# ushariRanasinghe/G2VLM

Measured on AMD Instinct MI355X. Metric: views/sec (multi-view recon, G2VLM-2B-MoT), higher is better.
Workload: dtype bf16; 1 GPU; C3: 8-view 518x518 reconstruction, full depth (24 DINO + 28 MoT + 15 decoder blocks), 1 scene per GPU; Lq=10968, Lk=10976, parallelism=replicas x1

## Files before the change

g2vlm_amd/csrc/gemm_8p.hip:

```cpp
#include <cstdlib>
#include "gemm_tile256.h"
#include "gemm_internal.h"

namespace {

typedef __attribute__((address_space(3))) void* lds_ptr_t;
typedef const __attribute__((address_space(1))) void* gbl_ptr_t;

template <int EPI, int MA0, int MA1, int PIPE>
__global__ __launch_bounds__(512, 2) void gemm8p_kernel(T256Args a) {
  constexpr int MT = MA0 + MA1;
  constexpr int HB = 16 * MT;
  constexpr int BMv = 2 * HB;
  constexpr int NA0 = (MA0 + 1) / 2, NA1 = (MA1 + 1) / 2;
  extern __shared__ __attribute__((aligned(16))) char smem[];

  const int tid = threadIdx.x, lane = tid & 63;
  const int w = __builtin_amdgcn_readfirstlane(tid >> 6);
  const int wr = w >> 2, wc = w & 3;
  const int N = a.N, K = a.K;
  const int srow = lane >> 3, scp = lane & 7;
  const int kcol = (scp ^ srow) << 3;
  int a_row[2][3], b_col[2][2], a_dst[2][3], b_dst[2][2];
#pragma unroll
  for (int q = 0; q < 2; ++q)
#pragma unroll
    for (int i2 = 0; i2 < 3; ++i2) {
      const int MA = q ? MA1 : MA0;
      int Lr = min(i2 * 64 + w * 8, 32 * MA - 8);
      a_row[q][i2] = (Lr / (16 * MA)) * HB + (q ? 16 * MA0 : 0) + Lr % (16 * MA);
      a_dst[q][i2] = a_row[q][i2] * 128;
    }
#pragma unroll
  for (int q = 0; q < 2; ++q)
#pragma unroll
    for (int i2 = 0; i2 < 2; ++i2) {
      int gq = w + 8 * i2;
      b_col[q][i2] = (gq >> 2) * 64 + q * 32 + (gq & 3) * 8;
      b_dst[q][i2] = OP_BYTES + b_col[q][i2] * 128;
    }

  struct TileCtx {
    int gi, m0, n0;
    uint32_t a_src[2][3], b_src[2][2];
  };
  auto setup_tile = [&](int vt, TileCtx& c) {
    tile_origin<BMv>(a, vt, c.gi, c.m0, c.n0);
    const int gM = a.g[c.gi].M;
#pragma unroll
    for (int q = 0; q < 2; ++q)
#pragma unroll
      for (int i2 = 0; i2 < 3; ++i2)
        c.a_src[q][i2] = ((uint32_t)(min(c.m0 + a_row[q][i2] + srow, gM - 1) - c.m0) * (uint32_t)a.lda + kcol) * 2u;
#pragma unroll
    for (int q = 0; q < 2; ++q)
#pragma unroll
      for (int i2 = 0; i2 < 2; ++i2)
        c.b_src[q][i2] = ((uint32_t)(min(c.n0 + b_col[q][i2] + srow, N - 1) - c.n0) * (uint32_t)K + kcol) * 2u;
  };
  auto stage_of = [&](int j, const __bf16* Ab, const __bf16* Wb, const uint32_t (&as)[2][3], const uint32_t (&bs)[2][2]) {
    const int t = j >> 2, c = j & 3;
    char* base = smem + (t & 1) * KBUF_BYTES;
    const char* Ak = reinterpret_cast<const char*>(Ab + t * BK);
    const char* Wk = reinterpret_cast<const char*>(Wb + t * BK);
    if (c == 0) {
#pragma unroll
      for (int i2 = 0; i2 < NA0; ++i2)
        if (i2 * 8 + w < 4 * MA0)
          __builtin_amdgcn_global_load_lds((gbl_ptr_t)(Ak + as[0][i2]), (lds_ptr_t)(base + a_dst[0][i2]), 16, 0, 0);
    } else if (c == 3) {
#pragma unroll
      for (int i2 = 0; i2 < NA1; ++i2)
        if (i2 * 8 + w < 4 * MA1)
          __builtin_amdgcn_global_load_lds((gbl_ptr_t)(Ak + as[1][i2]), (lds_ptr_t)(base + a_dst[1][i2]), 16, 0, 0);
    } else {
      const int q = c == 2;
#pragma unroll
      for (int i2 = 0; i2 < 2; ++i2)
        __builtin_amdgcn_global_load_lds((gbl_ptr_t)(Wk + bs[q][i2]), (lds_ptr_t)(base + b_dst[q][i2]), 16, 0, 0);
    }
  };

  TileCtx cur;
  setup_tile(blockIdx.x, cur);
  bool prefetched = false;
  for (int vt = blockIdx.x; vt < a.total; vt += gridDim.x) {
  const T256Group g = a.g[cur.gi];
  const int m0 = cur.m0, n0 = cur.n0, M = g.M;
  const __bf16* Abase = g.A + (size_t)m0 * a.lda;
  const __bf16* Wbase = g.W + (size_t)n0 * K;

  const int nk = K / BK;
  const int n_half = 4 * nk;
  auto stage = [&](int j) {
    if (j >= n_half || (prefetched && j < 4)) return;
    stage_of(j, Abase, Wbase, cur.a_src, cur.b_src);
  };
  auto wait_vm = [&](int n) {
    switch (n) {
      case 5: __builtin_amdgcn_s_waitcnt(0x0F75); break;
      case 6: __builtin_amdgcn_s_waitcnt(0x0F76); break;
      case 7: __builtin_amdgcn_s_waitcnt(0x0F77); break;
      case 8: __builtin_amdgcn_s_waitcnt(0x0F78); break;
      case 9: __builtin_amdgcn_s_waitcnt(0x0F79); break;
      default: __builtin_amdgcn_s_waitcnt(0x0F7A); break;
    }
  };
  const int cnt_a0 = (4 * MA0 - w + 7) >> 3, cnt_a1 = (4 * MA1 - w + 7) >> 3;
  auto wait_ring = [&]() { wait_vm(cnt_a0 + 4); };

  f32x4 acc[MT][4];
#pragma unroll
  for (int i = 0; i < MT; ++i)
#pragma unroll
    for (int j = 0; j < 4; ++j) acc[i][j] = f32x4{0.f, 0.f, 0.f, 0.f};

  const int fr = lane & 15, fq = lane >> 4;
  const int sw = (fq ^ (fr & 7)) << 4;
  const int aoff = (wr * HB + fr) * 128 + sw;
  const int boff = OP_BYTES + (wc * 64 + fr) * 128 + sw;

  bf16x8 fa[PIPE == 1 ? 2 : 1][MA0][2], fb[2][2][2];

  auto read_a = [&](const char* base, int qa) {
#pragma unroll
    for (int i = 0; i < (qa ? MA1 : MA0); ++i)
#pragma unroll
      for (int kk = 0; kk < 2; ++kk) {
#ifdef EXP_GEMM_HALF_LDS
        if (i & 1) { fa[PIPE == 1 ? qa : 0][i][kk] = fa[PIPE == 1 ? qa : 0][i - 1][kk]; continue; }
#endif
        fa[PIPE == 1 ? qa : 0][i][kk] = *reinterpret_cast<const bf16x8*>(base + ((aoff + (qa * 16 * MA0 + i * 16) * 128) ^ (kk << 6)));
      }
  };
  auto read_b = [&](const char* base, int qb) {
#pragma unroll
    for (int jj = 0; jj < 2; ++jj)
#pragma unroll
      for (int kk = 0; kk < 2; ++kk) {
#ifdef EXP_GEMM_HALF_LDS
        if (jj & 1) { fb[qb][jj][kk] = fb[qb][0][kk]; continue; }
#endif
        fb[qb][jj][kk] = *reinterpret_cast<const bf16x8*>(base + ((boff + qb * 4096 + jj * 2048) ^ (kk << 6)));
      }
  };
  const bool live = wr * HB < M - m0 || (a.flags & G2V_GEMM_8P_NO_ROW_SKIP);
  auto mma = [&](int qa, int qb) {
    if (!live) return;
#ifdef EXP_GEMM_NO_MFMA
#pragma unroll
    for (int kk = 0; kk < 2; ++kk) {
#pragma unroll
      for (int i = 0; i < (qa ? MA1 : MA0); ++i) acc[qa * MA0 + i][qb * 2][0] += (float)fa[PIPE == 1 ? qa : 0][i][kk][0];
#pragma unroll
      for (int jj = 0; jj < 2; ++jj) acc[qa * MA0][qb * 2 + jj][1] += (float)fb[qb][jj][kk][0];
    }
    return;
#endif
    __builtin_amdgcn_s_setprio(1);
#pragma unroll
    for (int kk = 0; kk < 2; ++kk)
#pragma unroll
      for (int i = 0; i < (qa ? MA1 : MA0); ++i)
#pragma unroll
        for (int jj = 0; jj < 2; ++jj)
          acc[qa * MA0 + i][qb * 2 + jj] =
              __builtin_amdgcn_mfma_f32_16x16x32_bf16(fb[qb][jj][kk], fa[PIPE == 1 ? qa : 0][i][kk], acc[qa * MA0 + i][qb * 2 + jj], 0, 0, 0);
    __builtin_amdgcn_s_setprio(0);
  };
  constexpr bool STAG = PIPE == 2;
  auto sync_lds = [&]() {
    if constexpr (STAG) {
      __builtin_amdgcn_s_waitcnt(0xC07F);
      __builtin_amdgcn_sched_barrier(0);
      __builtin_amdgcn_s_barrier();
    } else {
      __builtin_amdgcn_s_barrier();
      __builtin_amdgcn_s_waitcnt(0xC07F);
    }
    __builtin_amdgcn_sched_barrier(0);
  };

  if constexpr (PIPE != 1) {
    auto ktile = [&](int t) {
      const char* base = smem + (t & 1) * KBUF_BYTES;
      const int p = 4 * t;
      read_b(base, 0);
      __builtin_amdgcn_sched_barrier(0);
      read_a(base, 0);
      stage(p + 7);
      sync_lds();
      mma(0, 0);
      __builtin_amdgcn_s_barrier();
      read_b(base, 1);
      stage(p + 8);
      sync_lds();
      mma(0, 1);
      __builtin_amdgcn_s_barrier();
      read_a(base, 1);
      stage(p + 9);
      sync_lds();
      mma(1, 1);
      __builtin_amdgcn_s_barrier();
      stage(p + 10);
      if (t + 2 < nk) wait_ring();
      else __builtin_amdgcn_s_waitcnt(0x0F70);
      __builtin_amdgcn_s_barrier();
      mma(1, 0);
      __builtin_amdgcn_s_barrier();
    };

  #pragma unroll
    for (int j = 0; j < 7; ++j) stage(j);
    if (nk >= 2) wait_ring();
    else __builtin_amdgcn_s_waitcnt(0x0F70);
    __builtin_amdgcn_s_barrier();
    if constexpr (STAG) {
      if (wr == 1) __builtin_amdgcn_s_barrier();
    }

    for (int t = 0; t < nk; ++t) ktile(t);
    if constexpr (STAG) {
      if (wr == 0) __builtin_amdgcn_s_barrier();
    }
  } else {
    auto begin_phase = [&](bool retire, int t) {
      __builtin_amdgcn_s_waitcnt(0xC07F);
      if (retire && t + 1 < nk) {
        if (t + 2 < nk) wait_ring();
        else __builtin_amdgcn_s_waitcnt(0x0F70);
      }
      __builtin_amdgcn_sched_barrier(0);
      __builtin_amdgcn_s_barrier();
      __builtin_amdgcn_sched_barrier(0);
    };
#pragma unroll
    for (int j = 0; j < 8; ++j) stage(j);
    if (nk >= 2) {
      wait_vm(cnt_a0 + 4 + cnt_a1);
    } else {
      __builtin_amdgcn_s_waitcnt(0x0F70);
    }
    __builtin_amdgcn_s_barrier();
    read_a(smem, 0);
    read_b(smem, 0);
    __builtin_amdgcn_s_waitcnt(0xC07F);
    __builtin_amdgcn_s_barrier();
    stage(8);
    for (int t = 0; t < nk; ++t) {
      const char* base = smem + (t & 1) * KBUF_BYTES;
      const char* nbase = smem + ((t + 1) & 1) * KBUF_BYTES;
      const int p = 4 * t;
      begin_phase(false, t);
      stage(p + 9);
      read_b(base, 1);
      __builtin_amdgcn_sched_barrier(0);
      mma(0, 0);
      __builtin_amdgcn_sched_barrier(0);
      begin_phase(false, t);
      stage(p + 10);
      read_a(base, 1);
      __builtin_amdgcn_sched_barrier(0);
      mma(0, 1);
      __builtin_amdgcn_sched_barrier(0);
      begin_phase(true, t);
      stage(p + 11);
      read_a(nbase, 0);
      __builtin_amdgcn_sched_barrier(0);
      mma(1, 1);
      __builtin_amdgcn_sched_barrier(0);
      begin_phase(false, t);
      stage(p + 12);
      __builtin_amdgcn_sched_barrier(0);
      mma(1, 0);
      __builtin_amdgcn_sched_barrier(0);
      read_b(nbase, 0);
    }
    __builtin_amdgcn_s_waitcnt(0xC07F);
    __builtin_amdgcn_s_barrier();
  }

  const int vn = vt + gridDim.x;
  const bool has_next = vn < a.total;
  if (has_next) {
    setup_tile(vn, cur);
    const T256Group& gn_ = a.g[cur.gi];
    const __bf16* An = gn_.A + (size_t)cur.m0 * a.lda;
    const __bf16* Wn = gn_.W + (size_t)cur.n0 * K;
#pragma unroll
    for (int j = 0; j < 4; ++j) stage_of(j, An, Wn, cur.a_src, cur.b_src);
  }

#ifdef EXP_GEMM_NO_EPI
  {
    float sink = 0.f;
#pragma unroll
    for (int i = 0; i < MT; ++i)
#pragma unroll
      for (int j = 0; j < 4; ++j) sink += acc[i][j][0] + acc[i][j][1] + acc[i][j][2] + acc[i][j][3];
    if (sink == 1.2345e30f) reinterpret_cast<float*>(g.C)[tid] = sink;
    __builtin_amdgcn_s_barrier();
    prefetched = has_next;
    continue;
  }
#endif
  tile_epilogue<EPI, MT, 512, 4>(a, g, smem, tid, wr, wc, m0, n0, [&](auto i, auto j, auto r) { return acc[i.value][j.value][r.value]; });
  prefetched = has_next;
  }
}

template <int EPI, int MA0, int MA1, int PIPE>
int launch_h(const T256Args& a, hipStream_t s) { return launch_persistent<gemm8p_kernel<EPI, MA0, MA1, PIPE>, 512>(a, s); }

template <int EPI>
int launch(const T256Args& a, int bm, hipStream_t s) {
  if (a.flags & G2V_GEMM_8P_TWO_BARRIER) {
    if (bm == 288) return launch_h<EPI, 5, 4, 0>(a, s);
    if (bm == 256) return launch_h<EPI, 4, 4, 0>(a, s);
    if (bm == 224) return launch_h<EPI, 4, 3, 0>(a, s);
    if (bm == 192) return launch_h<EPI, 4, 2, 0>(a, s);
    if (bm == 160) return launch_h<EPI, 3, 2, 0>(a, s);
    return launch_h<EPI, 2, 2, 0>(a, s);
  }
  if (a.flags & G2V_GEMM_8P_PIPELINED) {
    if (bm == 288) return launch_h<EPI, 5, 4, 0>(a, s);
    if (bm == 256) return launch_h<EPI, 4, 4, 1>(a, s);
    if (bm == 224) return launch_h<EPI, 4, 3, 1>(a, s);
    if (bm == 192) return launch_h<EPI, 4, 2, 1>(a, s);
    if (bm == 160) return launch_h<EPI, 3, 2, 1>(a, s);
    return launch_h<EPI, 2, 2, 1>(a, s);
  }
  if (bm == 288) return launch_h<EPI, 5, 4, 2>(a, s);
  if (bm == 256) return launch_h<EPI, 4, 4, 2>(a, s);
  if (bm == 224) return launch_h<EPI, 4, 3, 2>(a, s);
  if (bm == 192) return launch_h<EPI, 4, 2, 2>(a, s);
  if (bm == 160) return launch_h<EPI, 3, 2, 2>(a, s);
  return launch_h<EPI, 2, 2, 2>(a, s);
}

}

static bool aligned16(const void* p) { return (reinterpret_cast<uintptr_t>(p) & 15) == 0; }

bool g2v_gemm_8p_supported(const g2v_gemm_desc* d) {
  if ((d->K % BK) || (d->N % BN) || (d->lda & 7) || d->K < 2 * BK) return false;
  if ((long)BM_MAX * d->lda >= (1L << 31) || (long)BN * d->K >= (1L << 31)) return false;
  const bool f32out = d->epilogue == G2V_EPI_RES_F32;
  if (d->ldc % (f32out ? 4 : 8)) return false;
  for (int i = 0; i < d->ngroups; ++i) {
    const g2v_gemm_group& g = d->g[i];
    if (g.M <= 0) continue;
    if (!aligned16(g.A) || !aligned16(g.W) || !aligned16(g.C)) return false;
    if (g.bias && (reinterpret_cast<uintptr_t>(g.bias) & 7)) return false;
    if (g.gamma && !aligned16(g.gamma)) return false;
    if (g.res && (!aligned16(g.res) || d->ldres % (f32out ? 4 : 8))) return false;
  }
  return true;
}

bool g2v_gemm_8p_preferred(const g2v_gemm_desc* d) {
  long rows = 0;
  for (int i = 0; i < d->ngroups; ++i) rows += d->g[i].M;
  return rows >= 1024 || (rows >= 256 && d->N >= 4096);
}

int g2v_gemm_8p_height(const g2v_gemm_desc* d) {
  const int tiles_n = d->N / BN;
  const int big = d->ngroups == 2 && d->g[1].M > d->g[0].M ? 1 : 0;
  const long m_big = d->g[big].M;
  const long m_small = d->ngroups == 2 ? d->g[1 - big].M : 0;
  int bm = 256;
  {
    double best = 1e30;
    const int hs[6] = {288, 256, 224, 192, 160, 128};
    const double hc[6] = {1.005, 1.0, 1.08, 1.12, 1.165, 1.23};
    for (int k = 0; k < 6; ++k) {
      const int h = hs[k];
      const int small_rows = m_small > 0 ? (int)((m_small + h - 1) / h) : 0;
      const long tiles = ((m_big + h - 1) / h + small_rows) * tiles_n;
      const long rounds = (tiles + 255) / 256;
      const double c = (double)rounds * h * hc[k];
      if (c < best) { best = c; bm = h; }
    }
  }
  if (d->flags & G2V_GEMM_8P_H192) bm = 192;
  if (d->flags & G2V_GEMM_8P_H128) bm = 128;
  if (d->flags & G2V_GEMM_8P_H256) bm = 256;
  if (d->flags & G2V_GEMM_8P_H288) bm = 288;
  if (d->flags & G2V_GEMM_8P_H224) bm = 224;
  if (d->flags & G2V_GEMM_8P_H160) bm = 160;
  return bm;
}

bool g2v_gemm_8p_four_waves(const g2v_gemm_desc* d) {
  if (d->flags & (G2V_GEMM_8P_EIGHT_WAVES | G2V_GEMM_8P_TWO_BARRIER | G2V_GEMM_8P_PIPELINED)) return false;
  static int mask = -1;
  if (mask < 0) {
    const char* e = getenv("G2V_GEMM_4W_MASK");
    mask = e ? atoi(e) : 6;
  }
  const int cls = d->N >= 8192 ? 1 : (d->K >= 4096 ? 2 : (d->epilogue == G2V_EPI_RES_F32 ? 4 : (d->epilogue == G2V_EPI_GELU ? 16 : 8)));
  return (d->flags & G2V_GEMM_8P_FOUR_WAVES) || (mask & cls);
}

int g2v_gemm_8p_launch(const g2v_gemm_desc* d, hipStream_t s) {
  const int bm = g2v_gemm_8p_height(d);
  T256Args a;
  a.ngroups = 0; a.N = d->N; a.K = d->K; a.lda = d->lda; a.ldc = d->ldc; a.ldres = d->ldres;
  a.tiles_n = d->N / BN; a.flags = d->flags;
  a.sn = a.tiles_n < 8 ? a.tiles_n : 8;
  a.sm = 32 / a.sn > 1 ? 32 / a.sn : 1;
  a.total = 0;
  const int big = d->ngroups == 2 && d->g[1].M > d->g[0].M;
  for (int i = 0; i < d->ngroups; ++i) {
    const g2v_gemm_group& sg = d->g[i ^ big];
    if (sg.M <= 0) continue;
    T256Group& g = a.g[a.ngroups++];
    g.A = (const __bf16*)sg.A; g.W = (const __bf16*)sg.W; g.bias = (const __bf16*)sg.bias; g.C = sg.C; g.res = sg.res;
    g.gamma = (const float*)sg.gamma; g.M = sg.M; g.tile_start = a.total;
    a.total += ((sg.M + bm - 1) / bm) * a.tiles_n;
  }
  if (a.ngroups == 1) a.g[1] = a.g[0];
  if (a.total == 0) return G2V_OK;
  if (g2v_gemm_8p_four_waves(d)) return g2v_gemm_4w_launch(a, d->epilogue, bm, s);
  return g2v_gemm_with_epilogue(d->epilogue, [&](auto epi) { return launch<decltype(epi)::value>(a, bm, s); });
}
```

g2vlm_amd/csrc/gemm_tile256.h:

```cpp
#pragma once
#include <type_traits>
#include <utility>
#include "common.h"
#include "g2vlm_hip.h"

struct T256Group {
  const __bf16* A; const __bf16* W; const __bf16* bias; void* C; const void* res; const float* gamma;
  int M, tile_start;
};
struct T256Args {
  T256Group g[2];
  int ngroups, N, K, lda, ldc, ldres, tiles_n, flags, sm, sn, total;
};

inline int g2v_persistent_cus() {
  static int n_cu = 0;
  if (n_cu == 0) {
    int dev = 0;
    hipDeviceProp_t prop;
    if (hipGetDevice(&dev) != hipSuccess || hipGetDeviceProperties(&prop, dev) != hipSuccess) return 0;
    n_cu = prop.multiProcessorCount & ~7;
    if (n_cu <= 0) n_cu = 256;
  }
  return n_cu;
}

namespace {

constexpr int BN = 256, BK = 64;
constexpr int BM_MAX = 288;
constexpr int OP_BYTES = BM_MAX * 128;
constexpr int KBUF_BYTES = OP_BYTES + 256 * 128;
constexpr int OUT_PITCH = 256 * 2 + 16;
constexpr int LDS_BYTES = KBUF_BYTES + 160 * OUT_PITCH;

template <class F, int... I>
__device__ __forceinline__ void sfor_impl(F&& f, std::integer_sequence<int, I...>) { (f(std::integral_constant<int, I>{}), ...); }
template <int N, class F>
__device__ __forceinline__ void sfor(F&& f) { sfor_impl(f, std::make_integer_sequence<int, N>{}); }

template <int BM>
__device__ __forceinline__ void tile_origin(const T256Args& a, int vt, int& gi, int& m0, int& n0) {
  const int nwg = a.total;
  int bid = vt;
  {
    int xcd = bid & 7, qn = nwg >> 3, rn = nwg & 7;
    bid = (xcd < rn ? xcd * (qn + 1) : rn * (qn + 1) + (xcd - rn) * qn) + (bid >> 3);
  }
  gi = (a.ngroups > 1 && bid >= a.g[1].tile_start) ? 1 : 0;
  const int t_id = bid - a.g[gi].tile_start;
  const int tiles_m = (a.g[gi].M + BM - 1) / BM;
  const int row_sz = a.sm * a.tiles_n;
  int sup_m = t_id / row_sz, r = t_id - sup_m * row_sz;
  int h = min(a.sm, tiles_m - sup_m * a.sm);
  int full_w = a.sn * h;
  int sup_n = r / full_w, p = r - sup_n * full_w;
  m0 = (sup_m * a.sm + p % h) * BM;
  n0 = (sup_n * a.sn + p / h) * BN;
}

template <int EPI, int MT, int NT, int NJ, class Acc>
__device__ __forceinline__ void tile_epilogue(const T256Args& a, const T256Group& g, char* smem, int tid, int wr, int wc, int m0, int n0, Acc&& acc) {
  constexpr bool SWI = EPI == G2V_EPI_SWIGLU;
  constexpr int HB = 16 * MT;
  constexpr int PITCH = OUT_PITCH;
  constexpr int I0 = (MT + 1) / 2;
  constexpr int CPR = SWI ? 16 : 32;
  constexpr int RPI = NT / CPR;
  const int M = g.M;
  char* const img = smem + KBUF_BYTES;
  int etid = tid;
  asm volatile("" : "+v"(etid));
  const int efr = etid & 15, efq = (etid >> 4) & 3;
  const int ch = etid % CPR, r0 = etid / CPR;
  const int gn = (SWI ? (n0 >> 1) : n0) + ch * 8;
  const bool round_gamma = a.flags & G2V_GEMM_GAMMA_ROUND_BF16;
  using OutT = std::conditional_t<EPI == G2V_EPI_RES_F32, float, __bf16>;
  const char* const rd = img + r0 * PITCH + ch * 16;
  OutT* const cl = reinterpret_cast<OutT*>(g.C) + gn;
  const OutT* const rl = reinterpret_cast<const OutT*>(g.res) + gn;
  sfor<2>([&](auto h_) {
    constexpr int h = h_;
    const int irow0 = wr * 16 * I0 + efr;
    if constexpr (SWI) {
      sfor<I0>([&](auto ii_) {
        constexpr int ii = ii_, i = h * I0 + ii;
        if constexpr (i < MT) {
          sfor<NJ / 2>([&](auto jp_) {
            constexpr int jp = jp_;
            float o[4];
            sfor<4>([&](auto r_) {
              constexpr int r = r_;
              float gt = bfround(acc(std::integral_constant<int, i>{}, std::integral_constant<int, 2 * jp>{}, r_));
              float up = bfround(acc(std::integral_constant<int, i>{}, std::integral_constant<int, 2 * jp + 1>{}, r_));
              float sl = bfround(siluf_fast_(gt));
              o[r] = sl * up;
            });
            *reinterpret_cast<u32x2*>(img + (irow0 + ii * 16) * PITCH + (wc * NJ * 8 + jp * 16 + efq * 4) * 2) =
                u32x2{pack_bf16x2(o[0], o[1]), pack_bf16x2(o[2], o[3])};
          });
        }
      });
    } else {
      sfor<NJ>([&](auto j_) {
        constexpr int j = j_;
        const int cl = wc * NJ * 16 + j * 16 + efq * 4;
        float bv[4] = {0.f, 0.f, 0.f, 0.f};
        if (g.bias) {
          u32x2 bb = *reinterpret_cast<const u32x2*>(g.bias + n0 + cl);
          bv[0] = bits2f_lo(bb[0]); bv[1] = bits2f_hi(bb[0]); bv[2] = bits2f_lo(bb[1]); bv[3] = bits2f_hi(bb[1]);
        }
        sfor<I0>([&](auto ii_) {
          constexpr int ii = ii_, i = h * I0 + ii;
          if constexpr (i < MT) {
            float o[4];
            sfor<4>([&](auto r_) {
              constexpr int r = r_;
              float v = bfround(acc(std::integral_constant<int, i>{}, j_, r_) + bv[r]);
              if constexpr (EPI == G2V_EPI_GELU) v = gelu_fast(v);
              if constexpr (EPI == G2V_EPI_QUICKGELU) {
                float u = bfround(1.702f * v);
                float sg = bfround(sigmoidf_(u));
                v = v * sg;
              }
              o[r] = v;
            });
            *reinterpret_cast<u32x2*>(img + (irow0 + ii * 16) * PITCH + cl * 2) = u32x2{pack_bf16x2(o[0], o[1]), pack_bf16x2(o[2], o[3])};
          }
        });
      });
    }
    float gam[8];
    bool has_gam = false;
    if constexpr (EPI == G2V_EPI_RES_F32) {
      has_gam = g.gamma != nullptr;
      if (has_gam) {
        f32x4 g0 = *reinterpret_cast<const f32x4*>(g.gamma + gn), g1 = *reinterpret_cast<const f32x4*>(g.gamma + gn + 4);
#pragma unroll
        for (int e = 0; e < 4; ++e) { gam[e] = g0[e]; gam[4 + e] = g1[e]; }
      }
    }
    __syncthreads();
    constexpr int NIT = 2 * 16 * I0 / RPI;
    constexpr int SB = NIT % 5 == 0 ? 5 : (NIT % 4 == 0 ? 4 : (NIT % 3 == 0 ? 3 : 2));
    static_assert(NIT % SB == 0, "sweep batches");
#pragma unroll
    for (int it0 = 0; it0 < NIT; it0 += SB) {
      u32x4 pk[SB];
      int gmv[SB];
      bool ok[SB];
      [[maybe_unused]] f32x4 ra[SB], rb[SB];
      [[maybe_unused]] u32x4 rr[SB];
#pragma unroll
      for (int c = 0; c < SB; ++c) {
        const int irow = (it0 + c) * RPI + r0;
        const int iwr = irow / (16 * I0), rem = irow - iwr * (16 * I0);
        const int trow = h * 16 * I0 + rem;
        gmv[c] = m0 + iwr * HB + trow;
        ok[c] = trow < HB && gmv[c] < M;
        if constexpr (EPI == G2V_EPI_RES_F32) {
          ra[c] = rb[c] = f32x4{0.f, 0.f, 0.f, 0.f};
          if (ok[c] && g.res) {
            const float* rp = rl + (size_t)gmv[c] * a.ldres;
            ra[c] = *reinterpret_cast<const f32x4*>(rp); rb[c] = *reinterpret_cast<const f32x4*>(rp + 4);
          }
        } else if constexpr (EPI == G2V_EPI_RES_BF16) {
          rr[c] = u32x4{0u, 0u, 0u, 0u};
          if (ok[c]) rr[c] = *reinterpret_cast<const u32x4*>(rl + (size_t)gmv[c] * a.ldres);
        }
      }
#pragma unroll
      for (int c = 0; c < SB; ++c) pk[c] = *reinterpret_cast<const u32x4*>(rd + (it0 + c) * RPI * PITCH);
#pragma unroll
      for (int c = 0; c < SB; ++c) {
        if (!ok[c]) continue;
        const int gm = gmv[c];
        if constexpr (EPI == G2V_EPI_RES_F32) {
          float v[8];
#pragma unroll
          for (int e = 0; e < 4; ++e) { v[2 * e] = bits2f_lo(pk[c][e]); v[2 * e + 1] = bits2f_hi(pk[c][e]); }
          if (has_gam) {
#pragma unroll
            for (int e = 0; e < 8; ++e) {
              v[e] = __fmul_rn(v[e], gam[e]);
              if (round_gamma) v[e] = bfround(v[e]);
            }
          }
          float* cp = cl + (size_t)gm * a.ldc;
          *reinterpret_cast<f32x4*>(cp) = f32x4{__fadd_rn(ra[c][0], v[0]), __fadd_rn(ra[c][1], v[1]), __fadd_rn(ra[c][2], v[2]), __fadd_rn(ra[c][3], v[3])};
          *reinterpret_cast<f32x4*>(cp + 4) = f32x4{__fadd_rn(rb[c][0], v[4]), __fadd_rn(rb[c][1], v[5]), __fadd_rn(rb[c][2], v[6]), __fadd_rn(rb[c][3], v[7])};
        } else if constexpr (EPI == G2V_EPI_RES_BF16) {
          u32x4 ov;
#pragma unroll
          for (int e = 0; e < 4; ++e)
            ov[e] = pack_bf16x2(bits2f_lo(rr[c][e]) + bits2f_lo(pk[c][e]), bits2f_hi(rr[c][e]) + bits2f_hi(pk[c][e]));
          *reinterpret_cast<u32x4*>(cl + (size_t)gm * a.ldc) = ov;
        } else {
          *reinterpret_cast<u32x4*>(cl + (size_t)gm * a.ldc) = pk[c];
        }
      }
    }
    __syncthreads();
  });
}

template <auto KERNEL, int NT>
int launch_persistent(const T256Args& a, hipStream_t s) {
  static bool attr_set = false;
  if (!attr_set) {
    if (hipFuncSetAttribute(reinterpret_cast<const void*>(KERNEL), hipFuncAttributeMaxDynamicSharedMemorySize, LDS_BYTES) != hipSuccess)
      return G2V_ERR_LAUNCH;
    attr_set = true;
  }
  const int n_cu = g2v_persistent_cus();
  if (n_cu == 0) return G2V_ERR_LAUNCH;
  hipLaunchKernelGGL(KERNEL, dim3(a.total < n_cu ? a.total : n_cu), dim3(NT), LDS_BYTES, s, a);
  G2V_CHECK_LAUNCH();
  return G2V_OK;
}

}
```

g2vlm_amd/hip.py:

```python
import ctypes as C
import os
import threading

import torch

_HERE = os.path.dirname(os.path.abspath(__file__))
LIB_PATH = os.environ.get("G2V_LIB_PATH") or os.path.join(_HERE, "lib", "libg2vlm_hip.so")

EPI_BF16, EPI_GELU, EPI_QUICKGELU, EPI_SWIGLU, EPI_RES_F32, EPI_RES_BF16 = range(6)
GAMMA_ROUND_BF16 = 1
FORCE_SMALL_TILE = 2
SUPERTILE = 4
FORCE_BIG_TILE = 8
FORCE_8P = 16
P8_H192, P8_H128, P8_H256, P8_TWO_BARRIER, P8_H288, P8_H224, P8_H160 = 128, 256, 512, 1024, 4096, 8192, 16384
P8_PIPELINED = 32768
P8_FOUR_WAVES = 65536
P8_EIGHT_WAVES = 131072
P8_NO_ROW_SKIP = 262144
F32, BF16 = 0, 1
NO_CAUSAL = 2 ** 30
_DEBUG_GEMM_FLAGS = int(os.environ.get("G2V_GEMM_FLAGS", "0"))


class GemmGroup(C.Structure):
    _fields_ = [("A", C.c_void_p), ("W", C.c_void_p), ("bias", C.c_void_p), ("C", C.c_void_p),
                ("res", C.c_void_p), ("gamma", C.c_void_p), ("M", C.c_int32), ("_pad", C.c_int32)]


class GemmDesc(C.Structure):
    _fields_ = [("g", GemmGroup * 2), ("ngroups", C.c_int32), ("N", C.c_int32), ("K", C.c_int32),
                ("lda", C.c_int32), ("ldc", C.c_int32), ("ldres", C.c_int32), ("epilogue", C.c_int32),
                ("flags", C.c_int32), ("workspace", C.c_void_p), ("workspace_bytes", C.c_int64)]


_P, _I, _F, _L = C.c_void_p, C.c_int, C.c_float, C.c_int64
_SIGS = {
    "g2v_version": ([], C.c_int),
    "g2v_arch": ([], C.c_char_p),
    "g2v_gemm_bf16": ([C.POINTER(GemmDesc), _P], C.c_int),
    "g2v_gemm_route": ([C.POINTER(GemmDesc), C.POINTER(C.c_int32 * 4)], C.c_int),
    "g2v_gemm_f32": ([_P, _P, _P, _P, _P, _I, _I, _I, _I, _I, _I, _I, _P], C.c_int),
    "g2v_layernorm": ([_P, _I, _I, _P, _P, _F, _P, _I, _I, _I, _I, _P], C.c_int),
    "g2v_rmsnorm": ([_P, _I, _P, _P, _I, _F, _P, _I, _I, _I, _I, _P], C.c_int),
    "g2v_mrope_table": ([_P, _I, _P, _P, _P, _P], C.c_int),
    "g2v_qknorm_mrope_cache": ([_P, _I, _I, _I, _P, _P, _P, _P, _I, _F, _I, _P, _P, _P, _P, _P, _P, _P], C.c_int),
    "g2v_flash_attn": ([_P, _I, _P, _I, _P, _I, _P, _I, _P, _I, _I, _I, _I, _F, _P, _P, _I, _P, _I, _I, _P, _P], C.c_int),
    "g2v_flash_attn_workspace": ([_I], C.c_int64),
    "g2v_debug_attn_form": ([_I], C.c_int),
    "g2v_rope2d": ([_P, _I, _I, _I, _I, _I, _P, _P, _P, _I, _P], C.c_int),
    "g2v_rope_vision": ([_P, _I, _I, _I, _I, _P, _P, _P], C.c_int),
    "g2v_im2col14": ([_P, _I, _I, _I, _P, _I, _P], C.c_int),
    "g2v_dino_preprocess": ([_P, _I, _I, _I, _I, C.POINTER(C.c_float), C.POINTER(C.c_float), _P, _P, _P], C.c_int),
    "g2v_dino_assemble": ([_P, _P, _P, _P, _P, _I, _I, _I, _P], C.c_int),
    "g2v_im2col_patch": ([_P, _I, _I, _I, _I, _P, _I, _P], C.c_int),
    "g2v_qwen_patchify_u8": ([_P, _I, _I, _I, C.POINTER(C.c_float), C.POINTER(C.c_float), _P, _I, _P], C.c_int),
    "g2v_vit_assemble": ([_P, _P, _P, _P, _I, _I, _I, _I, _P], C.c_int),
    "g2v_gather_rows_f32": ([_P, _I, _P, _P, _I, _I, _I, _P], C.c_int),
    "g2v_scatter_rows_f32": ([_P, _I, _P, _P, _I, _I, _I, _P], C.c_int),
    "g2v_cast_f32_bf16": ([_P, _P, _L, _P], C.c_int),
    "g2v_cast_bf16_f32": ([_P, _P, _L, _P], C.c_int),
    "g2v_pts_epilogue": ([_P, _I, _I, _I, _I, _P, _P, _P, _P], C.c_int),
    "g2v_pixel_shuffle14": ([_P, _I, _I, _I, _I, _P, _P], C.c_int),
    "g2v_lanczos_resize_u8": ([_P, _I, _I, _I, _P, _I, _I, _P, _P, _P, _I, _P, _P, _I, _P], C.c_int),
    "g2v_pts_epilogue_ps": ([_P, _I, _I, _I, _I, _I, _P, _P, _P, _P], C.c_int),
    "g2v_pixel_shuffle": ([_P, _I, _I, _I, _I, _I, _P, _P], C.c_int),
    "g2v_camera_tail": ([_P, _I, _I, _P, _P, _P, _P, _P, _P, _P, _P, _P, _P], C.c_int),
    "g2v_argmax_bf16": ([_P, _I, _P, _P, _P], C.c_int),
    "g2v_gemv_bf16": ([_P, _P, _P, _P, _P, _I, _I, _P], C.c_int),
    "g2v_decode_attn_workspace": ([_I, _I], C.c_int64),
    "g2v_gemv_rmsnorm_bf16": ([_P, _P, _F, _P, _P, _P, _I, _I, _P], C.c_int),
    "g2v_gemv_swiglu_bf16": ([_P, _P, _P, _I, _I, _P], C.c_int),
    "g2v_gemv_rmsnorm_swiglu_bf16": ([_P, _P, _F, _P, _P, _I, _I, _P], C.c_int),
    "g2v_decode_attn": ([_P, _P, _P, _P, _I, _I, _I, _F, _P, _P], C.c_int),
    "g2v_swiglu_bf16": ([_P, _P, _I, _P], C.c_int),
    "g2v_decode_attn_dyn": ([_P, _P, _P, _P, _P, _I, _I, _I, _F, _P, _P], C.c_int),
    "g2v_decode_advance": ([_P, _P, _P, _P], C.c_int),
    "g2v_decode_attn_batch": ([_P, _P, _P, _P, _P, _I, _L, _I, _I, _I, _F, _P, _P], C.c_int),
    "g2v_decode_advance_batch": ([_P, _P, _P, _I, _P], C.c_int),
    "g2v_decode_attn_fused": ([_P, _P, _P, _F, _I, _P, _P, _P, _P, _P, _P, _I, _L, _I, _I, _I, _F, _P, _P], C.c_int),
    "g2v_argmax_rows_bf16": ([_P, _I, _I, _L, _P, _P, _P], C.c_int),
    "g2v_gemv_pg": ([_P, _P, _F, _P, _P, _P, _P, _I, _I, _I, _P], C.c_int),
    "g2v_gemv_pg_batch": ([_P, _P, _F, _P, _P, _P, _P, _I, _I, _I, _I, _P], C.c_int),
    "g2v_decode_attn_pg_workspace": ([_I, _I, _I], C.c_int64),
    "g2v_decode_attn_pg": ([_P, _P, _P, _F, _I, _P, _P, _P, _P, _P, _P, _I, _L, _I, _I, _I, _F, _P, _P], C.c_int),
    "g2v_sample_rows_bf16": ([_P, _I, _I, _L, _P, _P, _P, _P], C.c_int),
    "g2v_decode_attn_shared_workspace": ([_I, _I, _I, _I, _I], C.c_int64),
    "g2v_decode_attn_shared": ([_P, _P, _P, _F, _I, _P, _P, _P, _P, _I, _P, _P, _P, _I, _L, _I, _I, _I, _F, _P, _P, _P], C.c_int),
    "g2v_gemv_pg_fp8": ([_P, _P, _F, _P, _P, _P, _P, _P, _I, _I, _I, _P], C.c_int),
    "g2v_gemv_pg_batch_fp8": ([_P, _P, _F, _P, _P, _P, _P, _P, _I, _I, _I, _I, _P], C.c_int),
    "g2v_gemv_pg_route": ([_I, _I, _I, _I, _I, _I, C.POINTER(C.c_int32 * 4)], C.c_int),
    "g2v_kv_quant_e4m3": ([_P, _L, _I, _P, _P, _P], C.c_int),
    "g2v_kv_dequant_e4m3": ([_P, _P, _L, _I, _P, _P], C.c_int),
    "g2v_decode_attn_pg_kv8": ([_P, _P, _P, _F, _I, _P, _P, _P, _P, _P, _P, _P, _P, _I, _L, _I, _I, _I, _F, _P, _P], C.c_int),
    "g2v_logprob_rows_workspace": ([_I, _I], C.c_int64),
    "g2v_logprob_rows_bf16": ([_P, _I, _I, _L, _P, _P, _P, _P, _P, _L, _P], C.c_int),
    "g2v_topk_rows_workspace": ([_I, _I, _I], C.c_int64),
    "g2v_topk_rows_bf16": ([_P, _I, _I, _L, _I, _P, _P, _P, _L, _P], C.c_int),
}
EXPORTS = tuple(_SIGS)

_lib = None


def lib():
    global _lib
    if _lib is None:
        if not os.path.exists(LIB_PATH):
            raise RuntimeError(f"{LIB_PATH} is missing: run `python -m g2vlm_amd.build` (hipcc, gfx950). "
                               "g2vlm_amd has no CPU fallback.")
        _lib = C.CDLL(LIB_PATH)
        for name, (args, res) in _SIGS.items():
            fn = getattr(_lib, name)
            fn.argtypes, fn.restype = args, res
        if torch.cuda.is_available():
            want = _lib.g2v_arch().decode()
            have = getattr(torch.cuda.get_device_properties(torch.cuda.current_device()), "gcnArchName", "")
            if have and not have.split(":")[0] == want:
                _lib = None
                raise RuntimeError(f"libg2vlm_hip.so is built for {want}; this device is {have}")
        if os.environ.get("G2V_ATTN_FORM"):
            _lib.g2v_debug_attn_form(int(os.environ["G2V_ATTN_FORM"]))
    return _lib


class HipError(RuntimeError):
    pass


def _ck(rc, what):
    if rc != 0:
        raise HipError(f"{what} failed with code {rc}")


_raw_stream = getattr(torch._C, "_cuda_getCurrentRawStream", None)


def _stream():
    if _raw_stream is not None:
        return C.c_void_p(_raw_stream(torch.cuda.current_device()))
    return C.c_void_p(torch.cuda.current_stream().cuda_stream)


def _p(t):
    if t is None:
        return None
    assert t.is_cuda, "libg2vlm_hip takes device pointers only"
    return C.c_void_p(t.data_ptr())


def _rowmajor(t):
    assert t.dim() == 2 and t.stride(1) == 1, "row-major 2-D view expected"
    return t.stride(0)


def h2d(t, device, dtype=None, resident=False):
    if t.is_cuda:
        return t.to(dtype) if dtype is not None else t
    if dtype is not None:
        t = t.to(dtype)
    if torch.device(device).type != "cuda":
        return t.to(device)
    out = t.contiguous().pin_memory().to(device, non_blocking=True)
    if resident:
        torch.cuda.current_stream(out.device).synchronize()
    return out


def scratch_owner(device_index):
    return (device_index, int(torch._C._cuda_getCurrentRawStream(device_index)), threading.get_ident())


# ... 648 lines not shown
```

include/g2vlm_hip.h:

```cpp
#ifndef G2VLM_HIP_H
#define G2VLM_HIP_H
#include <stdint.h>
#ifdef __cplusplus
extern "C" {
#endif

int g2v_version(void);
const char* g2v_arch(void);

enum {
  G2V_EPI_BF16 = 0,
  G2V_EPI_GELU = 1,
  G2V_EPI_QUICKGELU = 2,
  G2V_EPI_SWIGLU = 3,
  G2V_EPI_RES_F32 = 4,
  G2V_EPI_RES_BF16 = 5
};
#define G2V_GEMM_GAMMA_ROUND_BF16 1
#define G2V_GEMM_SUPERTILE 4
#define G2V_GEMM_FORCE_BIG_TILE 8
#define G2V_GEMM_FORCE_8P 16
#define G2V_GEMM_8P_H192 128
#define G2V_GEMM_8P_H128 256
#define G2V_GEMM_8P_H256 512
#define G2V_GEMM_8P_TWO_BARRIER 1024
#define G2V_GEMM_8P_H288 4096
#define G2V_GEMM_8P_H224 8192
#define G2V_GEMM_8P_H160 16384
#define G2V_GEMM_8P_PIPELINED 32768
#define G2V_GEMM_8P_FOUR_WAVES 65536
#define G2V_GEMM_8P_NO_ROW_SKIP 262144
#define G2V_GEMM_8P_EIGHT_WAVES 131072
#define G2V_GEMM_FORCE_SMALL_TILE 2

typedef struct {
  const void* A;
  const void* W;
  const void* bias;
  void* C;
  const void* res;
  const void* gamma;
  int32_t M;
  int32_t _pad;
} g2v_gemm_group;

typedef struct {
  g2v_gemm_group g[2];
  int32_t ngroups, N, K, lda, ldc, ldres, epilogue, flags;
  void* workspace;
  int64_t workspace_bytes;
} g2v_gemm_desc;

int g2v_gemm_bf16(const g2v_gemm_desc* desc, void* stream);
int g2v_gemm_route(const g2v_gemm_desc* desc, int32_t out[4]);

int g2v_gemm_f32(const void* A, const void* W, const void* bias, void* C, const void* res,
                 int M, int N, int K, int lda, int ldc, int ldres, int relu, void* stream);

#define G2V_F32 0
#define G2V_BF16 1
int g2v_layernorm(const void* x, int x_dtype, int ldx, const void* w, const void* b, float eps,
                  void* out, int out_dtype, int ldo, int M, int C, void* stream);
int g2v_rmsnorm(const void* x, int ldx, const void* w_lo, const void* w_hi, int split, float eps,
                void* out, int out_dtype, int ldo, int M, int C, void* stream);

int g2v_mrope_table(const void* pos, int L, const void* inv_freq , void* cos, void* sin, void* stream);
int g2v_qknorm_mrope_cache(const void* qkv, int L, int Hq, int Hkv,
                           const void* qw_lo, const void* qw_hi, const void* kw_lo, const void* kw_hi,
                           int split, float eps, int und_rounding, const void* cos, const void* sin,
                           void* q_out, void* k_cache, void* v_cache, const void* kv_rows, void* stream);

typedef struct {
  int32_t q0, q_rows;
  int32_t k0, k_len;
  int32_t causal_shift;
  int32_t q_win0;
  int32_t _pad[2];
} g2v_attn_tile;

typedef struct {
  int32_t desc;
  int32_t head;
  int32_t kt0, kt1;
  int32_t slot;
  int32_t _pad[3];
} g2v_attn_seg;
int64_t g2v_flash_attn_workspace(int n_slots);
int g2v_debug_attn_form(int form);
int g2v_flash_attn(const void* q, int ldq, const void* k, int ldk, const void* v, int ldv,
                   void* o, int ldo, const g2v_attn_tile* tiles, int n_tiles,
                   int Hq, int Hkv, int D, float scale,
                   const g2v_attn_seg* segs, const int32_t* seg_ptr, int n_blocks, const int32_t* comb, int n_comb,
                   int tile_rows, void* workspace, void* stream);

int g2v_rope2d(void* x, int ld, int M, int col0, int n_heads, int D, const void* cos, const void* sin,
               const void* pos, int P, void* stream);

int g2v_rope_vision(void* x, int ld, int M, int n_heads, int D, const void* cos, const void* sin, void* stream);

int g2v_dino_preprocess(const void* in, int in_is_u8, int N, int H, int W, const float* mean3, const float* std3, void* norm,
                        void* orig, void* stream);

int g2v_lanczos_resize_u8(const void* src, int N, int Hin, int Win, void* dst, int Hout, int Wout, void* tmp,
                          const void* bounds_h, const void* kk_h, int ksize_h,
                          const void* bounds_v, const void* kk_v, int ksize_v, void* stream);
int g2v_im2col14(const void* img, int N, int H, int W, void* out, int Kpad, void* stream);
int g2v_dino_assemble(const void* patch, const void* cls, const void* regs, const void* pos,
                      void* x, int N, int P, int C, void* stream);

int g2v_im2col_patch(const void* img, int N, int H, int W, int patch, void* out, int Kpad, void* stream);
int g2v_vit_assemble(const void* patch, const void* cls, const void* regs, void* x, int N, int P, int R, int C,
                     void* stream);

int g2v_qwen_patchify_u8(const void* img_u8, int F, int H, int W, const float* mean3, const float* std3, void* out,
                         int Kpad, void* stream);

int g2v_gather_rows_f32(const void* src, int ld_src, const void* idx, void* dst, int ld_dst,
                        int rows, int C, void* stream);
int g2v_scatter_rows_f32(const void* src, int ld_src, const void* idx, void* dst, int ld_dst,
                         int rows, int C, void* stream);
int g2v_cast_f32_bf16(const void* src, void* dst, int64_t n, void* stream);
int g2v_cast_bf16_f32(const void* src, void* dst, int64_t n, void* stream);

int g2v_pts_epilogue_ps(const void* feat, int N, int H, int W, int patch, int mode, const void* pose,
                        void* out, void* out2, void* stream);
int g2v_pts_epilogue(const void* feat, int N, int H, int W, int mode, const void* pose,
                     void* out, void* out2, void* stream);
int g2v_pixel_shuffle(const void* feat, int N, int H, int W, int C, int patch, void* out, void* stream);
int g2v_pixel_shuffle14(const void* feat, int N, int H, int W, int C, void* out, void* stream);

int g2v_camera_tail(const void* feat, int N, int P, const void* w0, const void* b0, const void* w1,
                    const void* b1, const void* wt, const void* bt, const void* wr, const void* br,
                    void* pose, void* stream);

int g2v_argmax_bf16(const void* x, int n, void* out, void* scratch, void* stream);


int g2v_gemv_bf16(const void* x, const void* W, const void* bias, void* out, void* res, int N, int K, void* stream);
int g2v_gemv_rmsnorm_bf16(const void* x_f32, const void* norm_w, float eps, const void* W, const void* bias, void* out,
                          int N, int K, void* stream);
int g2v_gemv_swiglu_bf16(const void* gu, const void* W, void* res, int N, int K, void* stream);
int g2v_gemv_rmsnorm_swiglu_bf16(const void* x_f32, const void* norm_w, float eps, const void* W_gu, void* act_out,
                                 int N2, int K, void* stream);
int g2v_swiglu_bf16(const void* gu, void* out, int n, void* stream);
int64_t g2v_decode_attn_workspace(int Lk, int Hq);
int g2v_decode_attn(const void* q, const void* k_cache, const void* v_cache, void* out, int Lk, int Hq,
                    int Hkv, float scale, void* workspace, void* stream);
int g2v_decode_attn_dyn(const void* q, const void* k_cache, const void* v_cache, void* out, const void* Lk_dev,
                        int max_len, int Hq, int Hkv, float scale, void* workspace, void* stream);
int g2v_decode_advance(void* pos3, void* row, void* len, void* stream);

int g2v_decode_attn_batch(const void* q, const void* k_cache, const void* v_cache, void* out, const void* Lk_dev,
                          int batch, int64_t scene_rows, int max_len, int Hq, int Hkv, float scale, void* workspace,
                          void* stream);
int g2v_decode_attn_fused(const void* qkv, const void* q_norm_w, const void* k_norm_w, float eps, int und_rounding,
                          const void* cos, const void* sin, void* k_cache, void* v_cache, void* out, const void* Lk_dev,
                          int batch, int64_t scene_rows, int max_len, int Hq, int Hkv, float scale, void* workspace,
                          void* stream);
int g2v_decode_advance_batch(void* pos3, void* row, void* len, int batch, void* stream);
int g2v_argmax_rows_bf16(const void* x, int rows, int n, int64_t ld, void* out, void* scratch, void* stream);
int g2v_sample_rows_bf16(const void* x, int rows, int n, int64_t ld, void* out, void* scratch, void* rng, void* stream);


int g2v_gemv_pg(const void* x, const void* norm_w, float eps, const void* W, const void* bias, void* out, void* res, int N,
                int K, int act, void* stream);
int g2v_gemv_pg_batch(const void* x, const void* norm_w, float eps, const void* W, const void* bias,
                      void* out, void* res, int B, int N, int K, int act, void* stream);

int g2v_gemv_pg_fp8(const void* x, const void* norm_w, float eps, const void* Wq, const void* wscale, const void* bias,
                    void* out, void* res, int N, int K, int act, void* stream);
int g2v_gemv_pg_batch_fp8(const void* x, const void* norm_w, float eps, const void* Wq, const void* wscale, const void* bias,
                          void* out, void* res, int B, int N, int K, int act, void* stream);

int g2v_gemv_pg_route(int B, int N, int K, int act, int norm, int fp8, int32_t out[4]);

int64_t g2v_decode_attn_pg_workspace(int Hq, int Hkv, int batch);
int g2v_decode_attn_pg(const void* qkv, const void* q_norm_w, const void* k_norm_w, float eps, int und_rounding,
                       const void* cos, const void* sin, void* k_cache, void* v_cache, void* out, const void* Lk_dev,
                       int batch, int64_t scene_rows, int max_len, int Hq, int Hkv, float scale, void* workspace, void* stream);

int64_t g2v_decode_attn_shared_workspace(int Hq, int Hkv, int batch, int prefix_len, int suffix_max_len);
int g2v_decode_attn_shared(const void* qkv, const void* q_norm_w, const void* k_norm_w, float eps, int und_rounding,
                           const void* cos, const void* sin, const void* k_prefix, const void* v_prefix, int prefix_len,
                           void* k_suffix, void* v_suffix, const void* suffix_len_dev, int batch, int64_t suffix_rows,
                           int suffix_max_len, int Hq, int Hkv, float scale, void* out, void* workspace, void* stream);
// ... 21 lines not shown
```

Before: 117.5 views/s.

## Defer GEMM epilogue global stores to overlap with next tile's prefetch

In the persistent 8-wave GEMM, full tiles with a following tile and a bias/GELU/SwiGLU epilogue now use a deferred epilogue. It stages the output tile through LDS into registers and issues stages 4-7 of the next tile's loads before the second half's global stores. The vmcnt waits in the first k-tile are widened to cover the outstanding stores, so stores drain while the next tile's loads and math proceed. This adds register pressure for the held output fragments and more complex waitcnt bookkeeping. The bias-load and image-write logic is refactored into a shared helper.

```diff
diff --git a/g2vlm_amd/csrc/gemm_8p.hip b/g2vlm_amd/csrc/gemm_8p.hip
--- a/g2vlm_amd/csrc/gemm_8p.hip
+++ b/g2vlm_amd/csrc/gemm_8p.hip
@@ -6,6 +6,87 @@
 
 typedef __attribute__((address_space(3))) void* lds_ptr_t;
 typedef const __attribute__((address_space(1))) void* gbl_ptr_t;
+
+#ifdef EXP_GEMM_DEFER_BOTH
+constexpr bool DEFER_BOTH_PASSES = true;
+#else
+constexpr bool DEFER_BOTH_PASSES = false;
+#endif
+template <int EPI, int MT, int H>
+constexpr int pass_stores() { return (H ? MT - (MT + 1) / 2 : (MT + 1) / 2) * (EPI == G2V_EPI_SWIGLU ? 1 : 2); }
+template <int EPI, int MT>
+constexpr int deferred_stores() { return pass_stores<EPI, MT, 1>() + (DEFER_BOTH_PASSES ? pass_stores<EPI, MT, 0>() : 0); }
+
+template <int EPI, int MT, class Acc, class StageNext>
+__device__ __forceinline__ void tile_epilogue_deferred(const T256Args& a, const T256Group& g, char* smem, int tid, int wr, int wc, int m0, int n0,
+                                                       Acc&& acc, StageNext&& stage_ktile1) {
+  constexpr bool SWI = EPI == G2V_EPI_SWIGLU;
+  constexpr int HB = 16 * MT, I0 = (MT + 1) / 2;
+  constexpr int CPR = SWI ? 16 : 32, RPI = 512 / CPR;
+  static_assert(pass_stores<EPI, MT, 0>() * RPI == 32 * I0 && pass_stores<EPI, MT, 1>() * RPI == 32 * (MT - I0), "sweeps cover each pass's rows exactly");
+  char* const img = smem + KBUF_BYTES;
+  int etid = tid;
+  asm volatile("" : "+v"(etid));
+  const int efr = etid & 15, efq = (etid >> 4) & 3;
+  const int ch = etid % CPR, r0 = etid / CPR;
+  __bf16* const cl = reinterpret_cast<__bf16*>(g.C) + (SWI ? (n0 >> 1) : n0) + ch * 8;
+  auto unpack = [](const u32x2& b, float (&bv)[4]) {
+    bv[0] = bits2f_lo(b[0]); bv[1] = bits2f_hi(b[0]); bv[2] = bits2f_lo(b[1]); bv[3] = bits2f_hi(b[1]);
+  };
+  auto lds_barrier = [&]() {
+    __builtin_amdgcn_s_waitcnt(0xC07F);
+    __builtin_amdgcn_sched_barrier(0);
+    __builtin_amdgcn_s_barrier();
+    __builtin_amdgcn_sched_barrier(0);
+  };
+  auto to_regs = [&](auto h_, auto& pk, auto&& bias, auto&& after_image) {
+    constexpr int H = h_.value, IH = H ? MT - I0 : I0;
+    tile_image_write<EPI, MT, 4, H>(img, wr, wc, efr, efq, acc, bias);
+    after_image();
+    lds_barrier();
+#pragma unroll
+    for (int it = 0; it < pass_stores<EPI, MT, H>(); ++it) {
+      const int lin = it * RPI + r0;
+      const int iwr = lin >= 16 * IH, rem = lin - iwr * 16 * IH;
+      pk[it] = *reinterpret_cast<const u32x4*>(img + (iwr * 16 * I0 + rem) * OUT_PITCH + ch * 16);
+    }
+#pragma unroll
+    for (int it = 0; it < pass_stores<EPI, MT, H>(); ++it) asm volatile("" : "+v"(pk[it]));
+    lds_barrier();
+  };
+  auto store = [&](auto h_, const auto& pk) {
+    constexpr int H = h_.value, IH = H ? MT - I0 : I0;
+#pragma unroll
+    for (int it = 0; it < pass_stores<EPI, MT, H>(); ++it) {
+      const int lin = it * RPI + r0;
+      const int iwr = lin >= 16 * IH, rem = lin - iwr * 16 * IH;
+      *reinterpret_cast<u32x4*>(cl + (size_t)(m0 + iwr * HB + H * 16 * I0 + rem) * a.ldc) = pk[it];
+    }
+  };
+  constexpr std::integral_constant<int, 0> P0{};
+  constexpr std::integral_constant<int, 1> P1{};
+  u32x4 pk0[pass_stores<EPI, MT, 0>()], pk1[pass_stores<EPI, MT, 1>()];
+  u32x2 bb[4] = {u32x2{0u, 0u}, u32x2{0u, 0u}, u32x2{0u, 0u}, u32x2{0u, 0u}};
+  to_regs(P0, pk0,
+          [&](auto, int c, float (&bv)[4]) {
+            if (g.bias) unpack(*reinterpret_cast<const u32x2*>(g.bias + n0 + c), bv);
+          },
+          [&]() {
+            if constexpr (!SWI) {
+              if (g.bias) {
+#pragma unroll
+                for (int j = 0; j < 4; ++j) bb[j] = *reinterpret_cast<const u32x2*>(g.bias + n0 + wc * 64 + j * 16 + efq * 4);
+#pragma unroll
+                for (int j = 0; j < 4; ++j) asm volatile("" : "+v"(bb[j]));
+              }
+            }
+          });
+  if constexpr (!DEFER_BOTH_PASSES) store(P0, pk0);
+  to_regs(P1, pk1, [&](auto j_, int, float (&bv)[4]) { unpack(bb[j_.value], bv); }, [] {});
+  stage_ktile1();
+  if constexpr (DEFER_BOTH_PASSES) store(P0, pk0);
+  store(P1, pk1);
+}
 
 template <int EPI, int MA0, int MA1, int PIPE>
 __global__ __launch_bounds__(512, 2) void gemm8p_kernel(T256Args a) {
@@ -84,6 +165,10 @@
   TileCtx cur;
   setup_tile(blockIdx.x, cur);
   bool prefetched = false;
+  bool deferred = false;
+  constexpr bool CAN_DEFER = PIPE != 1 && (EPI == G2V_EPI_BF16 || EPI == G2V_EPI_GELU || EPI == G2V_EPI_QUICKGELU || EPI == G2V_EPI_SWIGLU);
+  constexpr int S_LAST = deferred_stores<EPI, MT>();
+  static_assert(S_LAST + 10 <= 63, "vmcnt is a 6-bit counter");
   for (int vt = blockIdx.x; vt < a.total; vt += gridDim.x) {
   const T256Group g = a.g[cur.gi];
   const int m0 = cur.m0, n0 = cur.n0, M = g.M;
@@ -93,7 +178,7 @@
   const int nk = K / BK;
   const int n_half = 4 * nk;
   auto stage = [&](int j) {
-    if (j >= n_half || (prefetched && j < 4)) return;
+    if (j >= n_half || (prefetched && j < 4) || (deferred && j < 8)) return;
     stage_of(j, Abase, Wbase, cur.a_src, cur.b_src);
   };
   auto wait_vm = [&](int n) {
@@ -108,6 +193,20 @@
   };
   const int cnt_a0 = (4 * MA0 - w + 7) >> 3, cnt_a1 = (4 * MA1 - w + 7) >> 3;
   auto wait_ring = [&]() { wait_vm(cnt_a0 + 4); };
+  auto wait_vm_stores = [&](int n) {
+#define G2V_VMCNT(c) (0x0F70 | ((c) & 15) | (((c) >> 4) << 14))
+    switch (n) {
+      case 0: __builtin_amdgcn_s_waitcnt(G2V_VMCNT(S_LAST)); break;
+      case 5: __builtin_amdgcn_s_waitcnt(G2V_VMCNT(S_LAST + 5)); break;
+      case 6: __builtin_amdgcn_s_waitcnt(G2V_VMCNT(S_LAST + 6)); break;
+      case 7: __builtin_amdgcn_s_waitcnt(G2V_VMCNT(S_LAST + 7)); break;
+      case 8: __builtin_amdgcn_s_waitcnt(G2V_VMCNT(S_LAST + 8)); break;
+      case 9: __builtin_amdgcn_s_waitcnt(G2V_VMCNT(S_LAST + 9)); break;
+      case 10: __builtin_amdgcn_s_waitcnt(G2V_VMCNT(S_LAST + 10)); break;
+      default: __builtin_amdgcn_s_waitcnt(G2V_VMCNT(S_LAST)); break;
+    }
+#undef G2V_VMCNT
+  };
 
   f32x4 acc[MT][4];
 #pragma unroll
@@ -203,7 +302,8 @@
       mma(1, 1);
       __builtin_amdgcn_s_barrier();
       stage(p + 10);
-      if (t + 2 < nk) wait_ring();
+      if (CAN_DEFER && deferred && t == 0) wait_vm_stores(nk > 2 ? cnt_a0 + 4 : 0);
+      else if (t + 2 < nk) wait_ring();
       else __builtin_amdgcn_s_waitcnt(0x0F70);
       __builtin_amdgcn_s_barrier();
       mma(1, 0);
@@ -212,7 +312,8 @@
 
   #pragma unroll
     for (int j = 0; j < 7; ++j) stage(j);
-    if (nk >= 2) wait_ring();
+    if (CAN_DEFER && deferred) wait_vm_stores(cnt_a0 + 4 + cnt_a1);
+    else if (nk >= 2) wait_ring();
     else __builtin_amdgcn_s_waitcnt(0x0F70);
     __builtin_amdgcn_s_barrier();
     if constexpr (STAG) {
@@ -282,11 +383,12 @@
 
   const int vn = vt + gridDim.x;
   const bool has_next = vn < a.total;
+  const __bf16 *An = nullptr, *Wn = nullptr;
   if (has_next) {
     setup_tile(vn, cur);
     const T256Group& gn_ = a.g[cur.gi];
-    const __bf16* An = gn_.A + (size_t)cur.m0 * a.lda;
-    const __bf16* Wn = gn_.W + (size_t)cur.n0 * K;
+    An = gn_.A + (size_t)cur.m0 * a.lda;
+    Wn = gn_.W + (size_t)cur.n0 * K;
 #pragma unroll
     for (int j = 0; j < 4; ++j) stage_of(j, An, Wn, cur.a_src, cur.b_src);
   }
@@ -301,11 +403,24 @@
     if (sink == 1.2345e30f) reinterpret_cast<float*>(g.C)[tid] = sink;
     __builtin_amdgcn_s_barrier();
     prefetched = has_next;
+    deferred = false;
     continue;
   }
 #endif
-  tile_epilogue<EPI, MT, 512, 4>(a, g, smem, tid, wr, wc, m0, n0, [&](auto i, auto j, auto r) { return acc[i.value][j.value][r.value]; });
+  auto acc_of = [&](auto i, auto j, auto r) { return acc[i.value][j.value][r.value]; };
   prefetched = has_next;
+  deferred = false;
+  if constexpr (CAN_DEFER) {
+    deferred = has_next && m0 + BMv <= M && !(a.flags & G2V_GEMM_8P_OLD_BOUNDARY);
+    if (deferred) {
+      tile_epilogue_deferred<EPI, MT>(a, g, smem, tid, wr, wc, m0, n0, acc_of, [&]() {
+#pragma unroll
+        for (int j = 4; j < 8; ++j) stage_of(j, An, Wn, cur.a_src, cur.b_src);
+      });
+      continue;
+    }
+  }
+  tile_epilogue<EPI, MT, 512, 4>(a, g, smem, tid, wr, wc, m0, n0, acc_of);
   }
 }
 
diff --git a/g2vlm_amd/csrc/gemm_tile256.h b/g2vlm_amd/csrc/gemm_tile256.h
--- a/g2vlm_amd/csrc/gemm_tile256.h
+++ b/g2vlm_amd/csrc/gemm_tile256.h
@@ -57,6 +57,59 @@
   int sup_n = r / full_w, p = r - sup_n * full_w;
   m0 = (sup_m * a.sm + p % h) * BM;
   n0 = (sup_n * a.sn + p / h) * BN;
+}
+
+template <int EPI, int MT, int NJ, int H, class Acc, class Bias>
+__device__ __forceinline__ void tile_image_write(char* img, int wr, int wc, int efr, int efq, Acc&& acc, Bias&& bias) {
+  constexpr bool SWI = EPI == G2V_EPI_SWIGLU;
+  constexpr int PITCH = OUT_PITCH;
+  constexpr int I0 = (MT + 1) / 2;
+  const int irow0 = wr * 16 * I0 + efr;
+  if constexpr (SWI) {
+    sfor<I0>([&](auto ii_) {
+      constexpr int ii = ii_, i = H * I0 + ii;
+      if constexpr (i < MT) {
+        sfor<NJ / 2>([&](auto jp_) {
+          constexpr int jp = jp_;
+          float o[4];
+          sfor<4>([&](auto r_) {
+            constexpr int r = r_;
+            float gt = bfround(acc(std::integral_constant<int, i>{}, std::integral_constant<int, 2 * jp>{}, r_));
+            float up = bfround(acc(std::integral_constant<int, i>{}, std::integral_constant<int, 2 * jp + 1>{}, r_));
+            float sl = bfround(siluf_fast_(gt));
+            o[r] = sl * up;
+          });
+          *reinterpret_cast<u32x2*>(img + (irow0 + ii * 16) * PITCH + (wc * NJ * 8 + jp * 16 + efq * 4) * 2) =
+              u32x2{pack_bf16x2(o[0], o[1]), pack_bf16x2(o[2], o[3])};
+        });
+      }
+    });
+  } else {
+    sfor<NJ>([&](auto j_) {
+      constexpr int j = j_;
+      const int cl = wc * NJ * 16 + j * 16 + efq * 4;
+      float bv[4] = {0.f, 0.f, 0.f, 0.f};
+      bias(j_, cl, bv);
+      sfor<I0>([&](auto ii_) {
+        constexpr int ii = ii_, i = H * I0 + ii;
+        if constexpr (i < MT) {
+          float o[4];
+          sfor<4>([&](auto r_) {
+            constexpr int r = r_;
+            float v = bfround(acc(std::integral_constant<int, i>{}, j_, r_) + bv[r]);
+            if constexpr (EPI == G2V_EPI_GELU) v = gelu_fast(v);
+            if constexpr (EPI == G2V_EPI_QUICKGELU) {
+              float u = bfround(1.702f * v);
+              float sg = bfround(sigmoidf_(u));
+              v = v * sg;
+            }
+            o[r] = v;
+          });
+          *reinterpret_cast<u32x2*>(img + (irow0 + ii * 16) * PITCH + cl * 2) = u32x2{pack_bf16x2(o[0], o[1]), pack_bf16x2(o[2], o[3])};
+        }
+      });
+    });
+  }
 }
 
 template <int EPI, int MT, int NT, int NJ, class Acc>
@@ -81,55 +134,12 @@
   const OutT* const rl = reinterpret_cast<const OutT*>(g.res) + gn;
   sfor<2>([&](auto h_) {
     constexpr int h = h_;
-    const int irow0 = wr * 16 * I0 + efr;
-    if constexpr (SWI) {
-      sfor<I0>([&](auto ii_) {
-        constexpr int ii = ii_, i = h * I0 + ii;
-        if constexpr (i < MT) {
-          sfor<NJ / 2>([&](auto jp_) {
-            constexpr int jp = jp_;
-            float o[4];
-            sfor<4>([&](auto r_) {
-              constexpr int r = r_;
-              float gt = bfround(acc(std::integral_constant<int, i>{}, std::integral_constant<int, 2 * jp>{}, r_));
-              float up = bfround(acc(std::integral_constant<int, i>{}, std::integral_constant<int, 2 * jp + 1>{}, r_));
-              float sl = bfround(siluf_fast_(gt));
-              o[r] = sl * up;
-            });
-            *reinterpret_cast<u32x2*>(img + (irow0 + ii * 16) * PITCH + (wc * NJ * 8 + jp * 16 + efq * 4) * 2) =
-                u32x2{pack_bf16x2(o[0], o[1]), pack_bf16x2(o[2], o[3])};
-          });
-        }
-      });
-    } else {
-      sfor<NJ>([&](auto j_) {
-        constexpr int j = j_;
-        const int cl = wc * NJ * 16 + j * 16 + efq * 4;
-        float bv[4] = {0.f, 0.f, 0.f, 0.f};
-        if (g.bias) {
-          u32x2 bb = *reinterpret_cast<const u32x2*>(g.bias + n0 + cl);
-          bv[0] = bits2f_lo(bb[0]); bv[1] = bits2f_hi(bb[0]); bv[2] = bits2f_lo(bb[1]); bv[3] = bits2f_hi(bb[1]);
-        }
-        sfor<I0>([&](auto ii_) {
-          constexpr int ii = ii_, i = h * I0 + ii;
-          if constexpr (i < MT) {
-            float o[4];
-            sfor<4>([&](auto r_) {
-              constexpr int r = r_;
-              float v = bfround(acc(std::integral_constant<int, i>{}, j_, r_) + bv[r]);
-              if constexpr (EPI == G2V_EPI_GELU) v = gelu_fast(v);
-              if constexpr (EPI == G2V_EPI_QUICKGELU) {
-                float u = bfround(1.702f * v);
-                float sg = bfround(sigmoidf_(u));
-                v = v * sg;
-              }
-              o[r] = v;
-            });
-            *reinterpret_cast<u32x2*>(img + (irow0 + ii * 16) * PITCH + cl * 2) = u32x2{pack_bf16x2(o[0], o[1]), pack_bf16x2(o[2], o[3])};
-          }
-        });
-      });
-    }
+    tile_image_write<EPI, MT, NJ, h>(img, wr, wc, efr, efq, acc, [&](auto, int cl, float (&bv)[4]) {
+      if (g.bias) {
+        u32x2 bb = *reinterpret_cast<const u32x2*>(g.bias + n0 + cl);
+        bv[0] = bits2f_lo(bb[0]); bv[1] = bits2f_hi(bb[0]); bv[2] = bits2f_lo(bb[1]); bv[3] = bits2f_hi(bb[1]);
+      }
+    });
     float gam[8];
     bool has_gam = false;
     if constexpr (EPI == G2V_EPI_RES_F32) {
diff --git a/g2vlm_amd/hip.py b/g2vlm_amd/hip.py
--- a/g2vlm_amd/hip.py
+++ b/g2vlm_amd/hip.py
@@ -18,6 +18,7 @@
 P8_FOUR_WAVES = 65536
 P8_EIGHT_WAVES = 131072
 P8_NO_ROW_SKIP = 262144
+P8_OLD_BOUNDARY = 524288
 F32, BF16 = 0, 1
 NO_CAUSAL = 2 ** 30
 _DEBUG_GEMM_FLAGS = int(os.environ.get("G2V_GEMM_FLAGS", "0"))
diff --git a/include/g2vlm_hip.h b/include/g2vlm_hip.h
--- a/include/g2vlm_hip.h
+++ b/include/g2vlm_hip.h
@@ -31,6 +31,7 @@
 #define G2V_GEMM_8P_FOUR_WAVES 65536
 #define G2V_GEMM_8P_NO_ROW_SKIP 262144
 #define G2V_GEMM_8P_EIGHT_WAVES 131072
+#define G2V_GEMM_8P_OLD_BOUNDARY 524288
 #define G2V_GEMM_FORCE_SMALL_TILE 2
 
 typedef struct {
```

Result: no change. 118.2 views/s (median of 6 runs) (+0.6%).
